# wvangansbeke/LaneDetection_End2End

Measured on AMD Instinct MI355X. Metric: images/sec fwd+bwd, 256x512 2-lane bs32, higher is better.
Workload: dtype f32; 1 GPU; BEV ERFNet + fused WLS fit + Area loss, 2 lanes, 256x512, batch 32 per GPU, fp32, train mode (BN batch stats, Dropout2d on), fwd+bwd, optimizer excluded; global_batch=32, parallelism=dp1, grad_allreduce=none

## Files before the change

lanedetection_end2end_amd/_lib.py:

```python
import ctypes
import os
from ctypes import c_char_p, c_double, c_int, c_long, c_size_t, c_void_p

import torch

_HERE = os.path.dirname(os.path.abspath(__file__))
LIB_PATH = os.path.join(_HERE, "liblanefit_hip.so")
_lib = None


class LaneFitLibraryError(RuntimeError):
    pass


def _declare(lib):
    P, I, L, D = c_void_p, c_int, c_long, c_double
    sig = {
        "lf_abi_version": (c_int, []),
        "lf_last_error": (c_char_p, []),
        "lf_wls_workspace_bytes": (c_size_t, [I, I, I]),
        "lf_wls_fwd": (I, [P, P, L, I, I, I, I, I, I, D, D, I, I, P, P, P, P, P, P]),
        "lf_wls_bwd": (I, [P, P, L, I, I, I, I, I, I, D, I, P, P, P, P, P]),
        "lf_gels_workspace_bytes": (c_size_t, [I, I]),
        "lf_gels_fwd": (I, [P, P, I, L, I, P, P, P, P, P]),
# ... 86 lines not shown
        "lf_wls_bwd_theta": (I, [P, P, L, P, P, I, I, I, I, I, I, D, I, P, P, P, P, P, P, P]),
        "lf_wls_bwd_grid": (I, [P, P, L, I, I, I, I, I, I, D, I, P, P, P, P, P]),
    }
    dbg = {
        "lf_debug_set_split_any_size": (None, [I]),
        "lf_debug_set_bf16_lds": (None, [I]),
        "lf_debug_set_ops_precision": (None, [I]),
        "lf_debug_conv1d_fwd_phases": (I, [P, P, P, P, I, I, I, I, I, I, P, P, P]),
        "lf_debug_conv1d_wgrad_phases": (I, [P, P, I, I, I, I, I, I, P, P, P]),
        "lf_debug_conv1d_fwd_pro": (I, [P, P, P, P, P, P, I, I, I, I, I, I, P, P]),
        "lf_debug_set_wgrad_ro": (None, [I, I, I]),
        "lf_debug_conv1d_bwd_data_epi3": (I, [P, P, P, P, P, P, P, I, I, I, I, I, I, P, P]),
        "lf_debug_conv1d_epi": (I, [P, P, P, P, I, I, P, P, P, P, P, P, I, I, I, I, I, I, P, P]),
        "lf_debug_conv1d_wgrad_pro": (I, [P, P, P, P, P, P, I, I, I, I, I, I, P, P]),
        "lf_debug_bias_residual_launches": (L, []),
    }
    for table in (sig, dbg):
        for name, (res, args) in table.items():
            fn = getattr(lib, name)
            fn.restype = res
            fn.argtypes = args
    return sig


def exported_symbols():
    return list(_declare(load()).keys()) + list(_extra_symbols)


_extra_symbols = []

# ... 56 lines not shown
```

lanedetection_end2end_amd/csrc/lf_conv.h:

```cpp
#pragma once
#include "lf_common.h"

#define LF_MAX_TAPS 9

struct LfTapGeom {
    int N, Hl, Wl;
    int Hs, Ws, s_pix, s_choff;
    int ssh, ssw;
    int Hd, Wd, d_pix, d_choff;
    int dsh, dsw, dah, daw;
    int Cs, Cd;
    int ntaps;
    int tdh[LF_MAX_TAPS], tdw[LF_MAX_TAPS];
};

enum { LF_PRO_NONE = 0, LF_PRO_BNRELU = 1 };
enum {
    LF_EPI_RELU = 1,
    LF_EPI_MASK = 2,
    LF_EPI_ADD = 4,
    LF_EPI_STATS_SQ = 8,
    LF_EPI_MASKBN = 16,
    LF_EPI_STATS_XHAT = 32,
    LF_EPI_BIAS = 64
// ... 17 lines not shown
    const float* msh;
    const float* asc;
    const float* ash;
    const float* dm;
    float* stats;
    int stats_ld;
    unsigned long long* dbg;
};

void lf_tapgemm_set_split_any_size(int v);
void lf_tapgemm_set_bf16_lds(int v);
int lf_tapgemm_stat_rows(const LfTapGeom& g);
int lf_tapgemm_stat_rows_for(const LfTapGeom& g, const LfTapArgs& a);
int lf_tapgemm_launch(const LfTapGeom& g, const LfTapArgs& a, int pro, int epi, hipStream_t st);
int lf_tapgemm_launch_unordered(const LfTapGeom& g, const LfTapArgs& a, int pro, int epi, hipStream_t st);

struct LfWgradArgs {
    const float* x;
    const float* g;
    const float* pro_sc;
    const float* pro_sh;
    int s16;
    int split;
    float* partial;
    float* bias_partial;
    unsigned long long* dbg = nullptr;
};
int lf_tapwgrad_splits(const LfTapGeom& g);
int lf_tapwgrad_splits_bound(const LfTapGeom& g, int s16);
int lf_tapwgrad_splits_for(const LfTapGeom& g, const LfWgradArgs& a, int pro);
// ... 53 lines not shown
```

lanedetection_end2end_amd/csrc/lf_conv.hip:

```cpp
#include <stdlib.h>
#include <string.h>

#include <atomic>
#include <map>
#include <mutex>
#include <tuple>
#include <utility>

#include <hip/hip_ext.h>

#include "lf_conv.h"
#include "lf_ldsdma.h"
#include "lf_types.h"

typedef float f32x4 __attribute__((ext_vector_type(4)));

namespace {

constexpr int MT = 4;
constexpr int WG_WAVES = 4;
constexpr int PIX_PER_WG = WG_WAVES * MT * 16;

__device__ __forceinline__ f32x4 ldg4(const float* p) { return *reinterpret_cast<const f32x4*>(p); }
typedef unsigned u32x4v __attribute__((vector_size(16)));
// ... 54 lines not shown
    r.x = dpp_mov<0x150>(v.x); r.y = dpp_mov<0x150>(v.y); r.z = dpp_mov<0x150>(v.z); r.w = dpp_mov<0x150>(v.w);
    return r;
}
__device__ __forceinline__ float sum16(float v) {
    v += dpp_mov<0xB1>(v);
    v += dpp_mov<0x4E>(v);
    v += dpp_mov<0x124>(v);
    v += dpp_mov<0x128>(v);
    return v;
}

#define LF_EPI_GROUPS 1
#define LF_EPI_ONE_TILE false
#define LF_EPI_TID threadIdx.x
#define LF_EPI_ROW1 false
#define LF_EPI_PIVOT true
#define LF_TAPGEMM_EPILOGUE \
      \
    const bool stats = (epi & (LF_EPI_STATS_SQ | LF_EPI_STATS_XHAT)) != 0; \
    constexpr bool NOBIAS = EPIC >= 0 && !(EPIC & LF_EPI_BIAS) && (EPIC & (LF_EPI_MASK | LF_EPI_ADD | LF_EPI_MASKBN | LF_EPI_STATS_XHAT)) != 0; \
    constexpr int NC = (NT % 2 == 0 && !LF_EPI_ONE_TILE) ? 2 : 1; \
     \
    constexpr bool HOISTM = HOISTV && !(EPIC >= 0 && (EPIC & LF_EPI_MASKBN) && (EPIC & LF_EPI_STATS_XHAT)); \
    __builtin_amdgcn_s_setprio(3);    \
    const __amdgpu_buffer_rsrc_t r_dst = make_rsrc(a.dst, 0xffffffffu), r_add = make_rsrc(a.add_src, 0xffffffffu), \
                                 r_msk = make_rsrc(a.mask_src, 0xffffffffu), r_aux = make_rsrc(a.aux, 0xffffffffu), \
                                 r_bias = make_rsrc(a.bias, 0xffffffffu), r_msc = make_rsrc(a.msc, 0xffffffffu), \
                                 r_msh = make_rsrc(a.msh, 0xffffffffu), r_dm = make_rsrc(a.dm, 0xffffffffu); \
     \
    f32x4 s1[NT], s2[NT], bs[NOBIAS ? 1 : NT], hv[HOISTV ? NT : 1][2], piv[LF_EPI_PIVOT ? NT : 1]; \
// ... 52 lines not shown
        for (int n = 0; n < NT; ++n) { \
            const f32x4 dmv = ldb4(r_dm, (unsigned)(pn[0] * g.Cd + cob + n * 16 + kq * 4) * 4u, 0u); \
            s1[n] *= dmv; s2[n] *= dmv; \
        } \
    } \
    if (stats) { \
         \
        const int EW = wave & 3, EG = wave >> 2; \
        __shared__ float sred[LF_EPI_GROUPS][WG_WAVES][NT][4][8]; \
_Pragma("unroll") \
        for (int n = 0; n < NT; ++n) { \
            f32x4 r1, r2; \
            r1.x = sum16(s1[n].x); r1.y = sum16(s1[n].y); r1.z = sum16(s1[n].z); r1.w = sum16(s1[n].w); \
            r2.x = sum16(s2[n].x); r2.y = sum16(s2[n].y); r2.z = sum16(s2[n].z); r2.w = sum16(s2[n].w); \
            if (epi & LF_EPI_STATS_SQ) {       \
                const unsigned lf_t0 = (bx * (unsigned)(WG_WAVES * LF_EPI_GROUPS) + (unsigned)wave) * 64u; \
                const float nw = lf_t0 < npix ? (float)min(npix - lf_t0, 64u) : 0.f; \
                const float rn = nw > 0.f ? 1.f / nw : 0.f; \
                r2 = r2 - r1 * r1 * rn; \
                r2.x = fmaxf(r2.x, 0.f); r2.y = fmaxf(r2.y, 0.f); r2.z = fmaxf(r2.z, 0.f); r2.w = fmaxf(r2.w, 0.f); \
                if (LF_EPI_PIVOT) r1 = r1 + piv[LF_EPI_PIVOT ? n : 0] * nw; \
            } \
            if (pl == 0) { \
                float* d = sred[EG][EW][n][kq]; \
                d[0] = r1.x; d[1] = r1.y; d[2] = r1.z; d[3] = r1.w; d[4] = r2.x; d[5] = r2.y; d[6] = r2.z; d[7] = r2.w; \
            } \
        } \
        __syncthreads(); \
        if ((LF_EPI_TID & 255) < NT * 4 * 8) { \
            const int tg = LF_EPI_TID >> 8, tt = LF_EPI_TID & 255; \
            const int j = tt & 7, q = (tt >> 3) & 3, n = tt >> 5; \
            float v = sred[tg][0][n][q][j] + sred[tg][1][n][q][j] + sred[tg][2][n][q][j] + sred[tg][3][n][q][j]; \
            if ((epi & LF_EPI_STATS_SQ) && j >= 4) {       \
                const unsigned lf_tb = (bx * (unsigned)LF_EPI_GROUPS + (unsigned)tg) * (unsigned)(WG_WAVES * 64); \
                float nwv[4], sw[4], nt = 0.f, st = 0.f; \
_Pragma("unroll") \
                for (int w = 0; w < 4; ++w) { \
                    const unsigned t0w = lf_tb + (unsigned)w * 64u; \
                    nwv[w] = t0w < npix ? (float)min(npix - t0w, 64u) : 0.f; \
                    sw[w] = sred[tg][w][n][q][j - 4]; \
                    nt += nwv[w]; st += sw[w]; \
                } \
                const float mg = nt > 0.f ? st / nt : 0.f; \
_Pragma("unroll") \
                for (int w = 0; w < 4; ++w) \
                    if (nwv[w] > 0.f) { const float dmw = sw[w] / nwv[w] - mg; v += nwv[w] * dmw * dmw; } \
            } \
            const int co = cob + n * 16 + q * 4 + (j & 3); \
            a.stats[((long)(j >> 2) * g.Cd + co) * a.stats_ld + ((long)bx * LF_EPI_GROUPS + tg)] = v;       \
        } \
    } \

extern __shared__ __attribute__((aligned(16))) unsigned char lf_tap_lds[];
constexpr size_t LF_TAP_LDS_PER_TAP = (size_t)WG_WAVES * 64 * (sizeof(uint4) + sizeof(unsigned));
// ... 1553 lines not shown
                for (int n = 0; n < NT; ++n)
#pragma unroll
                    for (int m = 0; m < MT; ++m)
                        seg[n][m] = __builtin_amdgcn_mfma_f32_16x16x4f32(w[n][s], x[m][s], seg[n][m], 0, 0, 0);
        }
    }
    if (!(g.Cs == 16 && g.ntaps == 3)) {
#pragma unroll
        for (int n = 0; n < NT; ++n)
#pragma unroll
            for (int m = 0; m < MT; ++m) acc[n][m] += seg[n][m];
    }
    LF_TAPGEMM_EPILOGUE
}

int g_split_any_size = 0;
std::atomic<long> g_bres_launches{0};
int g_bf16_lds = 4;

int pick_nt(int Cd) {
    const int tiles = Cd / 16;
    if (tiles % 4 == 0) return 4;
    if (tiles % 3 == 0) return 3;
    if (tiles % 2 == 0) return 2;
    return 1;
}

}

void lf_tapgemm_set_split_any_size(int v) { g_split_any_size = v; }
long lf_tapgemm_bias_residual_launches() { return g_bres_launches.load(); }
void lf_tapgemm_set_bf16_lds(int v) { g_bf16_lds = v; }

bool lf_tapgemm_split_ok(const LfTapGeom& g) {
    const long npix = (long)g.N * g.Hl * g.Wl;
    const long wgs = npix / (2 * PIX_PER_WG) * (g.Cd / 64);
    return g.Cs % 32 == 0 && g.Cd % 64 == 0 && g.s_pix % 4 == 0 && g.s_choff % 4 == 0 && npix % (2 * PIX_PER_WG) == 0 &&
           (wgs >= 192 || g_split_any_size);
}

int lf_tapgemm_stat_rows(const LfTapGeom& g) {
    const long npix = (long)g.N * g.Hl * g.Wl;
    return lf_cdiv(npix, PIX_PER_WG);
}
int lf_tapgemm_stat_rows_for(const LfTapGeom& g, const LfTapArgs& a) {
    (void)a;
    return lf_cdiv((long)g.N * g.Hl * g.Wl, PIX_PER_WG);
// ... 291 lines not shown
            if (pro == LF_PRO_BNRELU && epi == LF_EPI_RELU) LF_TG4(1, LF_EPI_RELU);
            else if (pro == LF_PRO_BNRELU) LF_TG4(1, -1);
            else switch (epis) {
                case 0: LF_TG4(0, 0); break;
                case LF_EPI_RELU: LF_TG4(0, LF_EPI_RELU); break;
                case LF_EPI_MASK: LF_TG4(0, LF_EPI_MASK); break;
                case LF_EPI_ADD: LF_TG4(0, LF_EPI_ADD); break;
                case LF_EPI_STATS_SQ: LF_TG4(0, LF_EPI_STATS_SQ); break;
                case LF_EPI_MASK | LF_EPI_STATS_XHAT: LF_TG4(0, LF_EPI_MASK | LF_EPI_STATS_XHAT); break;
                case LF_EPI_ADD | LF_EPI_MASK | LF_EPI_STATS_XHAT: LF_TG4(0, LF_EPI_ADD | LF_EPI_MASK | LF_EPI_STATS_XHAT); break;
                case LF_EPI_MASKBN | LF_EPI_STATS_XHAT: LF_TG4(0, LF_EPI_MASKBN | LF_EPI_STATS_XHAT); break;
                case BRES: LF_TG4(0, BRES); ++g_bres_launches; break;
                default: LF_TG4(0, -1); break;
            }
            break;
        case 3: LF_TG(3); break;
        case 2: LF_TG(2); break;
        default:
            {
#define LF_LEAN(PROV, EPIV) hipLaunchKernelGGL((tapgemm_lean_kernel<1, PROV, EPIV>), grid, dim3(256), 0, st, g, a, pro, epi)
                if (pro == LF_PRO_BNRELU && epi == LF_EPI_RELU) LF_LEAN(1, LF_EPI_RELU);
                else if (pro == LF_PRO_BNRELU) LF_LEAN(1, -1);
                else switch (epis) {
                    case 0: LF_LEAN(0, 0); break;
                    case LF_EPI_RELU: LF_LEAN(0, LF_EPI_RELU); break;
                    case LF_EPI_MASK: LF_LEAN(0, LF_EPI_MASK); break;
                    case LF_EPI_ADD: LF_LEAN(0, LF_EPI_ADD); break;
                    case LF_EPI_STATS_SQ: LF_LEAN(0, LF_EPI_STATS_SQ); break;
                    case LF_EPI_MASK | LF_EPI_STATS_XHAT: LF_LEAN(0, LF_EPI_MASK | LF_EPI_STATS_XHAT); break;
                    case LF_EPI_ADD | LF_EPI_MASK | LF_EPI_STATS_XHAT: LF_LEAN(0, LF_EPI_ADD | LF_EPI_MASK | LF_EPI_STATS_XHAT); break;
                    case LF_EPI_MASKBN | LF_EPI_STATS_XHAT: LF_LEAN(0, LF_EPI_MASKBN | LF_EPI_STATS_XHAT); break;
                    case BRES: LF_LEAN(0, BRES); ++g_bres_launches; break;
                    default: LF_LEAN(0, -1); break;
                }
#undef LF_LEAN
            }
            break;
    }
#undef LF_TG
#undef LF_TG4
    LF_CHECK_LAUNCH("tapgemm");
    return 0;
}

namespace {

template <bool S16>
__device__ __forceinline__ f32x4 wg_ld4(__amdgpu_buffer_rsrc_t r, unsigned off) { return epi_ld<S16>(r, off); }
template <bool S16>
__device__ __forceinline__ float wg_ld1(__amdgpu_buffer_rsrc_t r, unsigned off, unsigned soff = 0u) {
    if constexpr (S16) return __uint_as_float((unsigned)__builtin_amdgcn_raw_buffer_load_b16(r, (int)(off * 2u), (int)(soff * 2u), 0) << 16);
    else return __builtin_bit_cast(float, __builtin_amdgcn_raw_buffer_load_b32(r, (int)(off * 4u), (int)(soff * 4u), 0));
}
__device__ __forceinline__ uint2 wg_ldraw(__amdgpu_buffer_rsrc_t r, unsigned off) {
    return __builtin_bit_cast(uint2, __builtin_amdgcn_raw_buffer_load_b64(r, (int)(off * 2u), 0, 0));
}
// ... 1092 lines not shown
```

lanedetection_end2end_amd/csrc/lf_debug.h:

```cpp
#pragma once
#ifdef __cplusplus
extern "C" {
#endif
void lf_debug_set_split_any_size(int v);
void lf_debug_set_bf16_lds(int v);
void lf_debug_set_ops_precision(int mode);
int lf_debug_conv1d_fwd_phases(const float* x, const float* w, const float* bias, float* y, int N, int H, int W, int C,
                               int axis, int dilation, float* scratch, unsigned long long* dbg, void* stream);
int lf_debug_conv1d_fwd_pro(const float* x, const float* w, const float* bias, const float* sc, const float* sh, float* y, int N, int H,
                            int W, int C, int axis, int dilation, float* scratch, void* stream);
void lf_debug_set_wgrad_ro(int mode, int cap64, int cap128);
int lf_debug_conv1d_wgrad_pro(const float* x, const float* gy, const float* sc, const float* sh, float* gw, float* gb, int N, int H, int W,
                              int C, int axis, int dilation, float* scratch, void* stream);
int lf_debug_conv1d_bwd_data_epi3(const float* gy, const float* w, const float* mask_src, const float* add_src, const float* aux,
                                  float* gx, float* stats, int N, int H, int W, int C, int axis, int dilation, float* scratch, void* stream);
int lf_debug_conv1d_epi(const float* src, const float* w, const float* bias, float* dst, int transposed, int epi, const float* mask_src,
                        const float* add_src, const float* aux, const float* msc, const float* msh, float* stats, int N, int H, int W, int C,
                        int axis, int dilation, float* scratch, void* stream);
long lf_debug_bias_residual_launches(void);
int lf_debug_conv1d_wgrad_phases(const float* x, const float* gy, int N, int H, int W, int C, int axis, int dilation,
                                 float* scratch, unsigned long long* dbg, void* stream);
#ifdef __cplusplus
}
#endif
// ... 1 lines not shown
```

lanedetection_end2end_amd/csrc/lf_erfnet.hip:

```cpp
#include <stdlib.h>

#include <vector>

#include "lf_conv.h"
#include "lf_eltwise.h"
#include "lf_plan.h"
#include "lf_types.h"

namespace {

constexpr float BN_EPS = 1e-3f, BN_MOM = 0.1f;
enum { K_DOWN = 0, K_NB = 1, K_UP = 2 };

struct GemmOp {
    LfTapGeom geom;
    int pack;
};
struct BNRef {
    int p_g, p_b, idx, C;
    long sc, sh, asc, ash, c1, c2;
};
struct ConvRef {
    int p_w, p_b;
    GemmOp fwd;
// ... 280 lines not shown
    };
    auto add_up = [&](int cin, int cout) {
        Layer L;
        memset(&L, 0, sizeof(L));
        L.kind = K_UP; L.Cin = cin; L.Cout = cout; L.Hin = h; L.Win = w; L.Hout = 2 * h; L.Wout = 2 * w; L.drop_idx = -1;
        L.x = cur; L.reg_lo = ws.cur;
        L.cv[0].p_w = param++; L.cv[0].p_b = param++;
        L.bn[0].p_g = param++; L.bn[0].p_b = param++; L.bn[0].idx = bn++; L.bn[0].C = cout;
        const long sz = (long)N * 2 * h * 2 * w * cout;
        L.b[0] = ws.take(sz); L.b[1] = ws.take(sz);
        bn_alloc(ws, L.bn[0]);
        build_up_conv(P, L.cv[0], N, h, w, cin, cout);
        long rows4 = 0;
        for (int ph = 0; ph < 4; ++ph) { rows4 += lf_tapgemm_stat_rows(L.cv[0].fph[ph].geom); account_wgrad(P, L.cv[0].fph[ph].geom); }
        P->stat_floats = lf_maxl(P->stat_floats, rows4 * 2 * cout);
        P->layers.push_back(L);
        cur = L.b[1]; h *= 2; w *= 2;
    };
    add_down(in_channels, 16);
    add_down(16, 64);
    for (int i = 0; i < 5; ++i) add_nb(64, 0.03f, 1);
    add_down(64, 128);
    const int dils[8] = {2, 4, 8, 16, 2, 4, 8, 16};
    for (int i = 0; i < 8; ++i) add_nb(128, 0.3f, dils[i]);
    param += 2;
    add_up(128, 64);
    add_nb(64, 0.f, 1); add_nb(64, 0.f, 1);
    add_up(64, 16);
    add_nb(16, 0.f, 1); add_nb(16, 0.f, 1);
    for (int i = 0; i < n_heads; ++i) { P->p_head_w[i] = param++; P->p_head_b[i] = param++; }
// ... 122 lines not shown

int run_gemm(const Ctx& c, const GemmOp& op, const float* src, float* dst, const float* bias, int pro, int epi,
             LfTapArgs extra, bool beside_wgrad = false) {
    extra.src = src; extra.dst = dst; extra.bias = bias; extra.wp = c.packed(op.pack);
    extra.s16 = c.s16;
    if (c.P->precision == 2)
        extra.wp16 = reinterpret_cast<const unsigned short*>(c.at(c.P->off_packed16)) + c.P->packs[op.pack].dst16_off;
    if (c.P->precision == 3) {
        extra.split = 9;
        extra.wp48 = reinterpret_cast<const unsigned short*>(c.at(c.P->off_packed48)) + 3 * c.P->packs[op.pack].dst16_off;
    }
    c.last_rows = lf_tapgemm_stat_rows_for(op.geom, extra);
    ProfScope ps(c, 0, op.geom, epi | (pro << 8), c.st);
    if (beside_wgrad && c.wgrad_launched && !c.P->prof_on) return lf_tapgemm_launch_unordered(op.geom, extra, pro, epi, c.st);
    return lf_tapgemm_launch(op.geom, extra, pro, epi, c.st);
}

int bn_finalize(const Ctx& c, const BNRef& b, const LfStatPart* parts, int nparts, double count) {
    return lf_bn_finalize_fwd(parts, nparts, b.C, count, c.params[b.p_g], c.params[b.p_b], c.running[2 * b.idx],
                              c.running[2 * b.idx + 1], BN_MOM, BN_EPS, c.training, c.at(b.sc), c.at(b.sh), c.at(b.asc),
                              c.at(b.ash), c.st);
}

int encoder_layers(const lf_erfnet_plan* P) {
    int n = 0;
    for (const Layer& L : P->layers) { if (L.kind == K_UP) break; ++n; }
    return n;
}

int forward_layers(const Ctx& c, const float* img, int nlayers, int first = 0) {
// ... 40 lines not shown
            a = lf_no_args();
            a.pro_sc = c.at(L.bn[0].sc); a.pro_sh = c.at(L.bn[0].sh);
            LF_TRY(run_gemm(c, L.cv[2].fwd, c.at(L.b[1]), c.at(L.b[2]), c.params[L.cv[2].p_b], LF_PRO_BNRELU, LF_EPI_RELU, a));
            a = lf_no_args();
            a.stats = stat0; a.stats_ld = lf_stat_ld(lf_tapgemm_stat_rows(L.cv[3].fwd.geom));
            LF_TRY(run_gemm(c, L.cv[3].fwd, c.at(L.b[2]), c.at(L.b[3]), c.params[L.cv[3].p_b], LF_PRO_NONE,
                            c.training ? LF_EPI_STATS_SQ : 0, a));
            p0.nrows = p0.seg_rows = c.last_rows; p0.ld = a.stats_ld;
            LF_TRY(bn_finalize(c, L.bn[1], &p0, 1, (double)npo));
            const float* dm = (c.training && L.drop_idx >= 0 && c.dropmask) ? c.dropmask + P->drop_off[L.drop_idx] : nullptr;
            LF_TRY(lf_bn_act(c.at(L.b[3]), c.at(L.bn[1].sc), c.at(L.bn[1].sh), dm, c.at(L.x), c.at(L.b[4]), npo, L.Cout,
                             (long)L.Hout * L.Wout, c.s16, c.st));
        } else {
            LfStatPart parts[1];
            int rows = 0, rows4 = 0;
            for (int ph = 0; ph < 4; ++ph) rows4 += lf_tapgemm_stat_rows(L.cv[0].fph[ph].geom);
            for (int ph = 0; ph < 4; ++ph) {
                LfTapArgs a = lf_no_args();
                a.stats = stat0 + rows; a.stats_ld = lf_stat_ld(rows4);
                LF_TRY(run_gemm(c, L.cv[0].fph[ph], c.at(L.x), c.at(L.b[0]), c.params[L.cv[0].p_b], LF_PRO_NONE,
                                c.training ? LF_EPI_STATS_SQ : 0, a));
                rows += c.last_rows;
            }
            parts[0] = lf_stat_part_tiles(stat0, rows, lf_stat_ld(rows4), L.Cout, 0, rows / 4, npo / 4);
            LF_TRY(bn_finalize(c, L.bn[0], parts, 1, (double)npo));
            LF_TRY(lf_bn_act(c.at(L.b[0]), c.at(L.bn[0].sc), c.at(L.bn[0].sh), nullptr, nullptr, c.at(L.b[1]), npo, L.Cout,
                             (long)L.Hout * L.Wout, c.s16, c.st));
        }
    }
    return 0;
}

struct BiasChain { float* base = nullptr; int rows = 0; int phase = 0; };

int run_wgrad(const Ctx& c, const GemmOp& op, const ConvRef& cv, const float* x, const float* g, const float* pro_sc,
              const float* pro_sh, int bias_accumulate, bool batch_off = false, BiasChain* chain = nullptr) {
    const lf_erfnet_plan* P = c.P;
    c.wgrad_launched = false;
    if (!c.grads[cv.p_w]) return 0;
// ... 192 lines not shown
            add_prep(a, epi, L.cv[0].dg[0].geom);
            LF_TRY(run_gemm(c, L.cv[0].dg[0], X, F, nullptr, LF_PRO_NONE, epi, a));
            out = F;
            if (can_prep) { prepped = true; prep_rows = c.last_rows; prep_ld = a.stats_ld; }
        } else if (L.x < 0) {
            const int Cc = 16 - L.Cin, rows = lf_stem_wgrad_rows(N, L.Hin, L.Win);
            if (c.grads[L.cv[0].p_w]) {
                const RowSums rs = row_sum_regions(c, (long)rows * Cc * L.Cin * 9, (long)rows * Cc);
                LF_TRY(lf_stem_wgrad(img, X, N, L.Cin, L.Hin, L.Win, rs.wrows, rs.brows, c.s16, c.st));
                LF_TRY(row_sums_finish(c, rs, rows, Cc * L.Cin * 9, c.grads[L.cv[0].p_w], Cc, c.grads[L.cv[0].p_b]));
            }
            out = F;
        } else {
            LF_TRY(run_wgrad(c, L.cv[0].fwd, L.cv[0], c.at(L.x), X, nullptr, nullptr, 0));
            LF_TRY(lf_pool_bwd(c.at(L.x), X, N, L.Hin, L.Win, L.Cin, L.Cout, L.Cout - L.Cin, F, c.s16, c.st));
            for (int ph = 0; ph < 4; ++ph) {
                LfTapArgs a = lf_no_args();
                a.add_src = F;
                LF_TRY(run_gemm(c, L.cv[0].dg[ph], X, F, nullptr, LF_PRO_NONE, LF_EPI_ADD, a));
            }
            out = F;
        }
        in = out;
    }
    if (gin) *gin = in;
    return 0;
}

int upload_and_pack(const Ctx& c, const float* const* params_dev) {
    const lf_erfnet_plan* P = c.P;
    LfPackEntry* ent = reinterpret_cast<LfPackEntry*>(c.at(P->off_entries));
// ... 440 lines not shown
```

lanedetection_end2end_amd/csrc/lf_ops.hip:

```cpp
#include "lf_conv.h"
#include "lf_debug.h"

namespace {

__global__ __launch_bounds__(256) void pack_one_kernel(const float* __restrict__ w, float* __restrict__ dst, int Kc, int Nc,
                                                      int ntaps, long sk, long sn, int flip) {
    const long total = (long)ntaps * Kc * Nc;
    for (long i = (long)blockIdx.x * 256 + threadIdx.x; i < total; i += (long)gridDim.x * 256) {
        const int k4 = (int)(i & 3);
        long r = i >> 2;
        const int n = (int)(r % Nc);
        r /= Nc;
        const int kb = (int)(r % (Kc >> 2));
        const int t = (int)(r / (Kc >> 2));
        dst[i] = w[(kb * 4 + k4) * sk + n * sn + (flip ? ntaps - 1 - t : t)];
    }
}

__global__ __launch_bounds__(256) void pack_one_bf16_kernel(const float* __restrict__ w, __bf16* __restrict__ dst, int Kc, int Nc,
                                                           int ntaps, long sk, long sn, int flip) {
    const int kb_per_tap = ((Kc + 31) >> 5) * 4;
    const long total = (long)ntaps * kb_per_tap * Nc * 8;
    for (long i = (long)blockIdx.x * 256 + threadIdx.x; i < total; i += (long)gridDim.x * 256) {
        const int k8 = (int)(i & 7);
// ... 36 lines not shown
            hipLaunchKernelGGL(pack_one_split_kernel, dim3(64), dim3(256), 0, st, w, reinterpret_cast<__bf16*>(scratch + 3L * C * C),
                               C, C, 3, sk, sn, flip);
            a.split = g_ops_bf16;
            a.wp48 = scratch + 3L * C * C;
        }
    } else if (g_ops_bf16 == 2) {
        hipLaunchKernelGGL(pack_one_bf16_kernel, dim3(64), dim3(256), 0, st, w, reinterpret_cast<__bf16*>(scratch), C, C, 3, sk, sn, flip);
        a.wp16 = scratch;
        a.s16 = 1;
    } else {
        hipLaunchKernelGGL(pack_one_kernel, dim3(64), dim3(256), 0, st, w, scratch, C, C, 3, sk, sn, flip);
    }
    a.wp = scratch;
}

LfTapGeom conv1d_geom(int N, int H, int W, int C, int axis, int d) {
    LfTapGeom g;
    memset(&g, 0, sizeof(g));
    g.N = N; g.Hl = H; g.Wl = W; g.Hs = H; g.Ws = W; g.s_pix = C; g.ssh = 1; g.ssw = 1;
    g.Hd = H; g.Wd = W; g.d_pix = C; g.dsh = 1; g.dsw = 1; g.Cs = C; g.Cd = C; g.ntaps = 3;
    for (int t = 0; t < 3; ++t) { g.tdh[t] = axis == 0 ? (t - 1) * d : 0; g.tdw[t] = axis == 1 ? (t - 1) * d : 0; }
    return g;
}

}

extern "C" {

void lf_debug_set_split_any_size(int v) { lf_tapgemm_set_split_any_size(v); }
void lf_debug_set_bf16_lds(int v) { lf_tapgemm_set_bf16_lds(v); }
void lf_debug_set_ops_precision(int mode) { g_ops_bf16 = (mode == 2 || mode == 9) ? mode : 0; }

void lf_debug_set_wgrad_ro(int mode, int cap64, int cap128) { lf_tapwgrad_ro_set(mode, cap64, cap128); }
long lf_debug_bias_residual_launches(void) { return lf_tapgemm_bias_residual_launches(); }

int lf_debug_conv1d_fwd_phases(const float* x, const float* w, const float* bias, float* y, int N, int H, int W, int C,
                               int axis, int dilation, float* scratch, unsigned long long* dbg, void* stream) {
    hipStream_t st = (hipStream_t)stream;
    const LfTapGeom g = conv1d_geom(N, H, W, C, axis, dilation);
    LfTapArgs a;
    memset(&a, 0, sizeof(a));
    pack_conv1d(a, w, scratch, C, 3L, 3L * C, 0, st);
    a.src = x; a.bias = bias; a.dst = y; a.dbg = dbg;
    return lf_tapgemm_launch(g, a, LF_PRO_NONE, 0, st);
}

// ... 116 lines not shown
```

Baseline: 1992 images/sec.

## Fuse four transposed-conv phase GEMMs into one kernel sharing input loads

Adds a phase4 kernel that computes all four sub-pixel phases of the stride-2 transposed convolution (upsampler) in one launch. It walks the 9 taps in an order that reuses each input pixel load across phases, and keeps four accumulator sets in registers. It is used for the forward pass with BN stats and for the backward data-grad with the add epilogue when fp32 and the geometry qualifies. It also specialises the 3-tap conv1d stats kernel on width alignment. The cost is higher register pressure from four accumulator sets, and separate stats tiling for the fused path.

New measurement: 2004 images/sec, median of 6. Within noise of the previous version (+0.6%).

```diff
diff --git a/lanedetection_end2end_amd/_lib.py b/lanedetection_end2end_amd/_lib.py
--- a/lanedetection_end2end_amd/_lib.py
+++ b/lanedetection_end2end_amd/_lib.py
@@ -124,6 +124,8 @@
         "lf_debug_conv1d_epi": (I, [P, P, P, P, I, I, P, P, P, P, P, P, I, I, I, I, I, I, P, P]),
         "lf_debug_conv1d_wgrad_pro": (I, [P, P, P, P, P, P, I, I, I, I, I, I, P, P]),
         "lf_debug_bias_residual_launches": (L, []),
+        "lf_debug_set_phase_fused": (None, [I]),
+        "lf_debug_phase4": (I, [P, P, P, P, P, P, I, I, I, I, I, I, I, P, P]),
     }
     for table in (sig, dbg):
         for name, (res, args) in table.items():
diff --git a/lanedetection_end2end_amd/csrc/lf_conv.h b/lanedetection_end2end_amd/csrc/lf_conv.h
--- a/lanedetection_end2end_amd/csrc/lf_conv.h
+++ b/lanedetection_end2end_amd/csrc/lf_conv.h
@@ -55,6 +55,13 @@
 int lf_tapgemm_stat_rows_for(const LfTapGeom& g, const LfTapArgs& a);
 int lf_tapgemm_launch(const LfTapGeom& g, const LfTapArgs& a, int pro, int epi, hipStream_t st);
 int lf_tapgemm_launch_unordered(const LfTapGeom& g, const LfTapArgs& a, int pro, int epi, hipStream_t st);
+
+struct LfPhase4 { unsigned woff[4]; int rows_per_phase; };
+bool lf_tapgemm_phase4_ok(const LfTapGeom* g, const LfTapArgs& a, const float* const* wp, int pro, int epi);
+int lf_tapgemm_phase4_tile_pix(const LfTapGeom& g0);
+int lf_tapgemm_phase4_stat_rows(const LfTapGeom& g0);
+int lf_tapgemm_phase4_launch(const LfTapGeom* g, const LfTapArgs& a, const float* const* wp, int epi, hipStream_t st);
+void lf_tapgemm_set_phase_fused(int v);
 
 struct LfWgradArgs {
     const float* x;
diff --git a/lanedetection_end2end_amd/csrc/lf_conv.hip b/lanedetection_end2end_amd/csrc/lf_conv.hip
--- a/lanedetection_end2end_amd/csrc/lf_conv.hip
+++ b/lanedetection_end2end_amd/csrc/lf_conv.hip
@@ -92,6 +92,7 @@
 #define LF_EPI_ONE_TILE false
 #define LF_EPI_TID threadIdx.x
 #define LF_EPI_ROW1 false
+#define LF_EPI_WPIX 64u
 #define LF_EPI_PIVOT true
 #define LF_TAPGEMM_EPILOGUE \
       \
@@ -174,8 +175,8 @@
             r1.x = sum16(s1[n].x); r1.y = sum16(s1[n].y); r1.z = sum16(s1[n].z); r1.w = sum16(s1[n].w); \
             r2.x = sum16(s2[n].x); r2.y = sum16(s2[n].y); r2.z = sum16(s2[n].z); r2.w = sum16(s2[n].w); \
             if (epi & LF_EPI_STATS_SQ) {       \
-                const unsigned lf_t0 = (bx * (unsigned)(WG_WAVES * LF_EPI_GROUPS) + (unsigned)wave) * 64u; \
-                const float nw = lf_t0 < npix ? (float)min(npix - lf_t0, 64u) : 0.f; \
+                const unsigned lf_t0 = (bx * (unsigned)(WG_WAVES * LF_EPI_GROUPS) + (unsigned)wave) * LF_EPI_WPIX; \
+                const float nw = lf_t0 < npix ? (float)min(npix - lf_t0, LF_EPI_WPIX) : 0.f; \
                 const float rn = nw > 0.f ? 1.f / nw : 0.f; \
                 r2 = r2 - r1 * r1 * rn; \
                 r2.x = fmaxf(r2.x, 0.f); r2.y = fmaxf(r2.y, 0.f); r2.z = fmaxf(r2.z, 0.f); r2.w = fmaxf(r2.w, 0.f); \
@@ -192,12 +193,12 @@
             const int j = tt & 7, q = (tt >> 3) & 3, n = tt >> 5; \
             float v = sred[tg][0][n][q][j] + sred[tg][1][n][q][j] + sred[tg][2][n][q][j] + sred[tg][3][n][q][j]; \
             if ((epi & LF_EPI_STATS_SQ) && j >= 4) {       \
-                const unsigned lf_tb = (bx * (unsigned)LF_EPI_GROUPS + (unsigned)tg) * (unsigned)(WG_WAVES * 64); \
+                const unsigned lf_tb = (bx * (unsigned)LF_EPI_GROUPS + (unsigned)tg) * ((unsigned)WG_WAVES * LF_EPI_WPIX); \
                 float nwv[4], sw[4], nt = 0.f, st = 0.f; \
 _Pragma("unroll") \
                 for (int w = 0; w < 4; ++w) { \
-                    const unsigned t0w = lf_tb + (unsigned)w * 64u; \
-                    nwv[w] = t0w < npix ? (float)min(npix - t0w, 64u) : 0.f; \
+                    const unsigned t0w = lf_tb + (unsigned)w * LF_EPI_WPIX; \
+                    nwv[w] = t0w < npix ? (float)min(npix - t0w, LF_EPI_WPIX) : 0.f; \
                     sw[w] = sred[tg][w][n][q][j - 4]; \
                     nt += nwv[w]; st += sw[w]; \
                 } \
@@ -1781,8 +1782,128 @@
     LF_TAPGEMM_EPILOGUE
 }
 
+template <int NTC, int EPIC>
+__global__ __launch_bounds__(256, 2) void tapgemm_phase4_kernel(const LfTapGeom g0, const LfTapArgs a0, const LfPhase4 pw) {
+    constexpr int NT = NTC, MT = 4 / NTC;
+    constexpr bool S16 = false, HOISTV = true;
+    const int epi = EPIC;
+    const int cob = 0;
+    const unsigned npix = (unsigned)(g0.N * g0.Hl * g0.Wl);
+    unsigned bx = blockIdx.x;
+    if ((gridDim.x & 7u) == 0) bx = (bx & 7u) * (gridDim.x >> 3) + (bx >> 3);
+    const int lane = threadIdx.x & 63, wave = threadIdx.x >> 6;
+    const int pl = lane & 15, kq = lane >> 4;
+    const unsigned tile0 = (bx * WG_WAVES + (unsigned)wave) * (MT * 16);
+    int pn[MT], pi[MT], pj[MT];
+    bool pv[MT];
+    unsigned xb[MT];
+#pragma unroll
+    for (int m = 0; m < MT; ++m) {
+        const unsigned p = tile0 + m * 16 + pl;
+        pv[m] = p < npix;
+        const unsigned q = pv[m] ? p : 0u;
+        const unsigned r = q / (unsigned)g0.Wl;
+        pj[m] = (int)(q - r * (unsigned)g0.Wl);
+        pn[m] = (int)(r / (unsigned)g0.Hl);
+        pi[m] = (int)(r - (unsigned)pn[m] * (unsigned)g0.Hl);
+        xb[m] = (unsigned)(((pn[m] * g0.Hs + pi[m]) * g0.Ws + pj[m]) * g0.s_pix + g0.s_choff + kq * 4) * 4u;
+    }
+    f32x4 accP[4][NT][MT], acclP[4][NT][MT];
+#pragma unroll
+    for (int ph = 0; ph < 4; ++ph)
+#pragma unroll
+        for (int n = 0; n < NT; ++n)
+#pragma unroll
+            for (int m = 0; m < MT; ++m) { accP[ph][n][m] = zero4(); acclP[ph][n][m] = zero4(); }
+    const int ncg = g0.Cs >> 4;
+    const __amdgpu_buffer_rsrc_t rx = make_rsrc(a0.src, (unsigned)min((long)g0.N * g0.Hs * g0.Ws * g0.s_pix * 4, (long)LF_OOB));
+    const __amdgpu_buffer_rsrc_t rw = make_rsrc(a0.wp, 0xffffffffu);
+    const unsigned wlane = (unsigned)(kq * g0.Cd + pl) * 16u;
+    const unsigned wstep = (unsigned)g0.Cd * 64u;
+#define LF_P4_XOFF(DST, DY, DX)                                                                              \
+    _Pragma("unroll") for (int m = 0; m < MT; ++m) {                                                          \
+        const bool in = pv[m] && pi[m] + (DY) < g0.Hs && pj[m] + (DX) < g0.Ws;                                \
+        DST[m] = in ? xb[m] + (unsigned)(((DY) * g0.Ws + (DX)) * g0.s_pix) * 4u : LF_OOB;                     \
+    }
+    f32x4 wc[NT], xc[MT];
+    {
+        unsigned xo[MT];
+        LF_P4_XOFF(xo, 1, 1)
+#pragma unroll
+        for (int n = 0; n < NT; ++n) wc[n] = ldb4(rw, wlane + n * 256, pw.woff[3]);
+#pragma unroll
+        for (int m = 0; m < MT; ++m) xc[m] = ldb4(rx, xo[m], 0u);
+    }
+#define LF_P4_TAP(PH, TAPI, DY, DX, PHN, TAPIN, DYN, DXN)                                                     \
+    {                                                                                                         \
+        unsigned xo[MT], xon[MT];                                                                             \
+        LF_P4_XOFF(xo, DY, DX)                                                                                \
+        LF_P4_XOFF(xon, DYN, DXN)                                                                             \
+        const unsigned wb = pw.woff[PH] + (unsigned)((TAPI) * ncg) * wstep;                                   \
+        const unsigned wbn = pw.woff[PHN] + (unsigned)((TAPIN) * ncg) * wstep;                                \
+        for (int cg = 0; cg < ncg; ++cg) {                                                                    \
+            const bool last = cg + 1 == ncg;                                                                  \
+            const unsigned wso = last ? wbn : wb + (unsigned)(cg + 1) * wstep;                                \
+            const unsigned c16 = last ? 0u : (unsigned)(cg + 1) * 64u;                                        \
+            f32x4 wn[NT], xn[MT];                                                                             \
+            _Pragma("unroll") for (int n = 0; n < NT; ++n) wn[n] = ldb4(rw, wlane + n * 256, wso);            \
+            _Pragma("unroll") for (int m = 0; m < MT; ++m) xn[m] = ldb4(rx, last ? xon[m] : xo[m], c16);      \
+            if (!(cg & 1)) {       \
+                _Pragma("unroll") for (int n = 0; n < NT; ++n)                                                \
+                    _Pragma("unroll") for (int m = 0; m < MT; ++m) {                                          \
+                        acclP[PH][n][m] += accP[PH][n][m];                                                    \
+                        accP[PH][n][m] = zero4();                                                             \
+                    }                                                                                         \
+            }                                                                                                 \
+            _Pragma("unroll") for (int s4 = 0; s4 < 4; ++s4)                                                  \
+                _Pragma("unroll") for (int n = 0; n < NT; ++n)                                                \
+                    _Pragma("unroll") for (int m = 0; m < MT; ++m)                                            \
+                        accP[PH][n][m] = __builtin_amdgcn_mfma_f32_16x16x4f32(wc[n][s4], xc[m][s4], accP[PH][n][m], 0, 0, 0); \
+            _Pragma("unroll") for (int n = 0; n < NT; ++n) wc[n] = wn[n];                                     \
+            _Pragma("unroll") for (int m = 0; m < MT; ++m) xc[m] = xn[m];                                     \
+        }                                                                                                     \
+    }
+    LF_P4_TAP(3, 0, 1, 1, 3, 1, 1, 0)
+    LF_P4_TAP(3, 1, 1, 0, 2, 0, 1, 0)
+    LF_P4_TAP(2, 0, 1, 0, 3, 2, 0, 1)
+    LF_P4_TAP(3, 2, 0, 1, 1, 0, 0, 1)
+    LF_P4_TAP(1, 0, 0, 1, 3, 3, 0, 0)
+    LF_P4_TAP(3, 3, 0, 0, 2, 1, 0, 0)
+    LF_P4_TAP(2, 1, 0, 0, 1, 1, 0, 0)
+    LF_P4_TAP(1, 1, 0, 0, 0, 0, 0, 0)
+    LF_P4_TAP(0, 0, 0, 0, 0, 0, 0, 0)
+#undef LF_P4_TAP
+#undef LF_P4_XOFF
+#pragma unroll
+    for (int ph = 0; ph < 4; ++ph)
+#pragma unroll
+        for (int n = 0; n < NT; ++n)
+#pragma unroll
+            for (int m = 0; m < MT; ++m) accP[ph][n][m] += acclP[ph][n][m];
+#undef LF_EPI_WPIX
+#define LF_EPI_WPIX ((unsigned)(MT * 16))
+#define LF_P4_EPI(PH)                                                                                         \
+    {                                                                                                         \
+        LfTapGeom g = g0;                                                                                     \
+        g.dah = (PH) >> 1; g.daw = (PH) & 1;                                                                  \
+        LfTapArgs a = a0;                                                                                     \
+        a.stats = a0.stats + (long)(PH) * pw.rows_per_phase;                                                  \
+        f32x4 (&acc)[NT][MT] = accP[PH];                                                                      \
+        LF_TAPGEMM_EPILOGUE                                                                                   \
+    }
+    LF_P4_EPI(0)
+    LF_P4_EPI(1)
+    LF_P4_EPI(2)
+    LF_P4_EPI(3)
+#undef LF_P4_EPI
+#undef LF_EPI_WPIX
+#define LF_EPI_WPIX 64u
+    __builtin_amdgcn_s_setprio(0);
+}
+
 int g_split_any_size = 0;
 std::atomic<long> g_bres_launches{0};
+int g_phase_fused = 1;
 int g_bf16_lds = 4;
 
 int pick_nt(int Cd) {
@@ -1798,6 +1919,7 @@
 void lf_tapgemm_set_split_any_size(int v) { g_split_any_size = v; }
 long lf_tapgemm_bias_residual_launches() { return g_bres_launches.load(); }
 void lf_tapgemm_set_bf16_lds(int v) { g_bf16_lds = v; }
+void lf_tapgemm_set_phase_fused(int v) { g_phase_fused = v; }
 
 bool lf_tapgemm_split_ok(const LfTapGeom& g) {
     const long npix = (long)g.N * g.Hl * g.Wl;
@@ -2119,7 +2241,12 @@
                 default: LF_TG4(0, -1); break;
             }
             break;
-        case 3: LF_TG(3); break;
+        case 3:
+            if (pro == LF_PRO_NONE && epis == LF_EPI_STATS_SQ) {
+                if ((g.Wl & 63) == 0) launch_tapgemm(tapgemm_kernel<3, 0, LF_EPI_STATS_SQ, true>, grid, tap_lds, st, g, a, pro, epi);
+                else launch_tapgemm(tapgemm_kernel<3, 0, LF_EPI_STATS_SQ, false>, grid, tap_lds, st, g, a, pro, epi);
+            } else LF_TG(3);
+            break;
         case 2: LF_TG(2); break;
         default:
             {
@@ -2145,6 +2272,50 @@
 #undef LF_TG
 #undef LF_TG4
     LF_CHECK_LAUNCH("tapgemm");
+    return 0;
+}
+
+int lf_tapgemm_phase4_tile_pix(const LfTapGeom& g0) { return g0.Cd == 64 ? 64 : 256; }
+int lf_tapgemm_phase4_stat_rows(const LfTapGeom& g0) { return lf_cdiv((long)g0.N * g0.Hl * g0.Wl, lf_tapgemm_phase4_tile_pix(g0)); }
+bool lf_tapgemm_phase4_ok(const LfTapGeom* g, const LfTapArgs& a, const float* const* wp, int pro, int epi) {
+    if (!g_phase_fused || a.s16 || a.wp16 || a.split || a.dbg || pro != LF_PRO_NONE) return false;
+    if (!(epi == 0 || epi == LF_EPI_STATS_SQ || (epi == LF_EPI_ADD && !a.bias))) return false;
+    const LfTapGeom& g0 = g[0];
+    if (!((g0.Cd == 64 && g0.Cs % 32 == 0) || (g0.Cd == 16 && g0.Cs % 16 == 0)) || g0.Wl % 16 != 0) return false;
+    if (g0.s_pix % 4 || g0.s_choff % 4 || g0.d_pix % 4 || g0.d_choff % 4) return false;
+    if ((long)g0.N * g0.Hs * g0.Ws * g0.s_pix * 4 >= (long)LF_OOB || (long)g0.N * g0.Hd * g0.Wd * g0.d_pix * 4 >= (long)LF_OOB) return false;
+    if ((long)g0.N * g0.Hl * g0.Wl >= (1L << 30)) return false;
+    static const int ntap[4] = {1, 2, 2, 4};
+    static const int dy[4][4] = {{0}, {0, 0}, {1, 0}, {1, 1, 0, 0}}, dx[4][4] = {{0}, {1, 0}, {0, 0}, {1, 0, 1, 0}};
+    for (int ph = 0; ph < 4; ++ph) {
+        const LfTapGeom& p = g[ph];
+        if (p.N != g0.N || p.Hl != g0.Hl || p.Wl != g0.Wl || p.Hs != p.Hl || p.Ws != p.Wl || p.ssh != 1 || p.ssw != 1 || p.dsh != 2 ||
+            p.dsw != 2 || p.Hd != 2 * p.Hl || p.Wd != 2 * p.Wl || p.dah != (ph >> 1) || p.daw != (ph & 1) || p.s_pix != g0.s_pix ||
+            p.s_choff != g0.s_choff || p.d_pix != g0.d_pix || p.d_choff != g0.d_choff || p.Cs != g0.Cs || p.Cd != g0.Cd || p.ntaps != ntap[ph])
+            return false;
+        for (int t = 0; t < p.ntaps; ++t)
+            if (p.tdh[t] != dy[ph][t] || p.tdw[t] != dx[ph][t]) return false;
+        if (wp[ph] < wp[0] || (wp[ph] - wp[0]) * 4L >= (1L << 30)) return false;
+    }
+    return true;
+}
+int lf_tapgemm_phase4_launch(const LfTapGeom* g, const LfTapArgs& a0, const float* const* wp, int epi, hipStream_t st) {
+    LfTapArgs a = a0;
+    LF_REQUIRE(lf_tapgemm_phase4_ok(g, a, wp, LF_PRO_NONE, epi), "tapgemm_phase4: launch not qualified (geometry, epilogue %d or precision)", epi);
+    LfPhase4 pw;
+    for (int ph = 0; ph < 4; ++ph) pw.woff[ph] = (unsigned)((wp[ph] - wp[0]) * 4L);
+    pw.rows_per_phase = lf_tapgemm_phase4_stat_rows(g[0]);
+    a.wp = wp[0];
+    const dim3 grid(pw.rows_per_phase);
+#define LF_P4(NTV)                                                                                                              \
+    do {                                                                                                                        \
+        if (epi == 0) hipLaunchKernelGGL((tapgemm_phase4_kernel<NTV, 0>), grid, dim3(256), 0, st, g[0], a, pw);                  \
+        else if (epi == LF_EPI_ADD) hipLaunchKernelGGL((tapgemm_phase4_kernel<NTV, LF_EPI_ADD>), grid, dim3(256), 0, st, g[0], a, pw); \
+        else hipLaunchKernelGGL((tapgemm_phase4_kernel<NTV, LF_EPI_STATS_SQ>), grid, dim3(256), 0, st, g[0], a, pw);             \
+    } while (0)
+    if (g[0].Cd == 64) LF_P4(4); else LF_P4(1);
+#undef LF_P4
+    LF_CHECK_LAUNCH("tapgemm_phase4");
     return 0;
 }
 
diff --git a/lanedetection_end2end_amd/csrc/lf_debug.h b/lanedetection_end2end_amd/csrc/lf_debug.h
--- a/lanedetection_end2end_amd/csrc/lf_debug.h
+++ b/lanedetection_end2end_amd/csrc/lf_debug.h
@@ -4,6 +4,9 @@
 #endif
 void lf_debug_set_split_any_size(int v);
 void lf_debug_set_bf16_lds(int v);
+void lf_debug_set_phase_fused(int v);
+int lf_debug_phase4(const float* src, const float* w, const float* bias, float* dst, const float* add_src, float* stats, int epi, int N,
+                    int H, int W, int Ck, int Cn, int s_pix, float* scratch, void* stream);
 void lf_debug_set_ops_precision(int mode);
 int lf_debug_conv1d_fwd_phases(const float* x, const float* w, const float* bias, float* y, int N, int H, int W, int C,
                                int axis, int dilation, float* scratch, unsigned long long* dbg, void* stream);
diff --git a/lanedetection_end2end_amd/csrc/lf_erfnet.hip b/lanedetection_end2end_amd/csrc/lf_erfnet.hip
--- a/lanedetection_end2end_amd/csrc/lf_erfnet.hip
+++ b/lanedetection_end2end_amd/csrc/lf_erfnet.hip
@@ -318,6 +318,7 @@
         long rows4 = 0;
         for (int ph = 0; ph < 4; ++ph) { rows4 += lf_tapgemm_stat_rows(L.cv[0].fph[ph].geom); account_wgrad(P, L.cv[0].fph[ph].geom); }
         P->stat_floats = lf_maxl(P->stat_floats, rows4 * 2 * cout);
+        P->stat_floats = lf_maxl(P->stat_floats, 4L * lf_tapgemm_phase4_stat_rows(L.cv[0].fph[0].geom) * 2 * cout);
         P->layers.push_back(L);
         cur = L.b[1]; h *= 2; w *= 2;
     };
@@ -470,6 +471,22 @@
     ProfScope ps(c, 0, op.geom, epi | (pro << 8), c.st);
     if (beside_wgrad && c.wgrad_launched && !c.P->prof_on) return lf_tapgemm_launch_unordered(op.geom, extra, pro, epi, c.st);
     return lf_tapgemm_launch(op.geom, extra, pro, epi, c.st);
+}
+
+int run_phase4(const Ctx& c, const GemmOp* ops, const float* src, float* dst, const float* bias, int epi, LfTapArgs extra, bool* fused) {
+    *fused = false;
+    if (c.P->precision != 0) return 0;
+    extra.src = src; extra.dst = dst; extra.bias = bias; extra.s16 = c.s16;
+    LfTapGeom g[4];
+    const float* wp[4];
+    for (int ph = 0; ph < 4; ++ph) { g[ph] = ops[ph].geom; wp[ph] = c.packed(ops[ph].pack); }
+    if (!lf_tapgemm_phase4_ok(g, extra, wp, LF_PRO_NONE, epi)) return 0;
+    *fused = true;
+    LfTapGeom gp = g[0];
+    gp.ntaps = 9;
+    c.last_rows = 4 * lf_tapgemm_phase4_stat_rows(g[0]);
+    ProfScope ps(c, 0, gp, epi, c.st);
+    return lf_tapgemm_phase4_launch(g, extra, wp, epi, c.st);
 }
 
 int bn_finalize(const Ctx& c, const BNRef& b, const LfStatPart* parts, int nparts, double count) {
@@ -540,15 +557,23 @@
         } else {
             LfStatPart parts[1];
             int rows = 0, rows4 = 0;
+            bool fused = false;
+            {
+                LfTapArgs a = lf_no_args();
+                a.stats = stat0; a.stats_ld = lf_stat_ld(4 * lf_tapgemm_phase4_stat_rows(L.cv[0].fph[0].geom));
+                LF_TRY(run_phase4(c, L.cv[0].fph, c.at(L.x), c.at(L.b[0]), c.params[L.cv[0].p_b], c.training ? LF_EPI_STATS_SQ : 0, a, &fused));
+                if (fused) parts[0] = lf_stat_part_tiles(stat0, c.last_rows, a.stats_ld, L.Cout, 0, c.last_rows / 4, npo / 4,
+                                                         lf_tapgemm_phase4_tile_pix(L.cv[0].fph[0].geom));
+            }
             for (int ph = 0; ph < 4; ++ph) rows4 += lf_tapgemm_stat_rows(L.cv[0].fph[ph].geom);
-            for (int ph = 0; ph < 4; ++ph) {
+            for (int ph = 0; ph < 4 && !fused; ++ph) {
                 LfTapArgs a = lf_no_args();
                 a.stats = stat0 + rows; a.stats_ld = lf_stat_ld(rows4);
                 LF_TRY(run_gemm(c, L.cv[0].fph[ph], c.at(L.x), c.at(L.b[0]), c.params[L.cv[0].p_b], LF_PRO_NONE,
                                 c.training ? LF_EPI_STATS_SQ : 0, a));
                 rows += c.last_rows;
             }
-            parts[0] = lf_stat_part_tiles(stat0, rows, lf_stat_ld(rows4), L.Cout, 0, rows / 4, npo / 4);
+            if (!fused) parts[0] = lf_stat_part_tiles(stat0, rows, lf_stat_ld(rows4), L.Cout, 0, rows / 4, npo / 4);
             LF_TRY(bn_finalize(c, L.bn[0], parts, 1, (double)npo));
             LF_TRY(lf_bn_act(c.at(L.b[0]), c.at(L.bn[0].sc), c.at(L.bn[0].sh), nullptr, nullptr, c.at(L.b[1]), npo, L.Cout,
                              (long)L.Hout * L.Wout, c.s16, c.st));
@@ -771,7 +796,13 @@
         } else {
             LF_TRY(run_wgrad(c, L.cv[0].fwd, L.cv[0], c.at(L.x), X, nullptr, nullptr, 0));
             LF_TRY(lf_pool_bwd(c.at(L.x), X, N, L.Hin, L.Win, L.Cin, L.Cout, L.Cout - L.Cin, F, c.s16, c.st));
-            for (int ph = 0; ph < 4; ++ph) {
+            bool fused = false;
+            {
+                LfTapArgs a = lf_no_args();
+                a.add_src = F;
+                LF_TRY(run_phase4(c, L.cv[0].dg, X, F, nullptr, LF_EPI_ADD, a, &fused));
+            }
+            for (int ph = 0; ph < 4 && !fused; ++ph) {
                 LfTapArgs a = lf_no_args();
                 a.add_src = F;
                 LF_TRY(run_gemm(c, L.cv[0].dg[ph], X, F, nullptr, LF_PRO_NONE, LF_EPI_ADD, a));
diff --git a/lanedetection_end2end_amd/csrc/lf_ops.hip b/lanedetection_end2end_amd/csrc/lf_ops.hip
--- a/lanedetection_end2end_amd/csrc/lf_ops.hip
+++ b/lanedetection_end2end_amd/csrc/lf_ops.hip
@@ -74,6 +74,21 @@
     a.wp = scratch;
 }
 
+__global__ __launch_bounds__(256) void pack_taps_kernel(const float* __restrict__ w, float* __restrict__ dst, int Kc, int Nc, int ntaps,
+                                                       long sk, long sn, int4 tapidx) {
+    const long total = (long)ntaps * Kc * Nc;
+    for (long i = (long)blockIdx.x * 256 + threadIdx.x; i < total; i += (long)gridDim.x * 256) {
+        const int k4 = (int)(i & 3);
+        long r = i >> 2;
+        const int n = (int)(r % Nc);
+        r /= Nc;
+        const int kb = (int)(r % (Kc >> 2));
+        const int t = (int)(r / (Kc >> 2));
+        const int ti = t == 0 ? tapidx.x : t == 1 ? tapidx.y : t == 2 ? tapidx.z : tapidx.w;
+        dst[i] = w[(kb * 4 + k4) * sk + n * sn + ti];
+    }
+}
+
 LfTapGeom conv1d_geom(int N, int H, int W, int C, int axis, int d) {
     LfTapGeom g;
     memset(&g, 0, sizeof(g));
@@ -90,6 +105,48 @@
 void lf_debug_set_split_any_size(int v) { lf_tapgemm_set_split_any_size(v); }
 void lf_debug_set_bf16_lds(int v) { lf_tapgemm_set_bf16_lds(v); }
 void lf_debug_set_ops_precision(int mode) { g_ops_bf16 = (mode == 2 || mode == 9) ? mode : 0; }
+
+void lf_debug_set_phase_fused(int v) { lf_tapgemm_set_phase_fused(v); }
+
+int lf_debug_phase4(const float* src, const float* w, const float* bias, float* dst, const float* add_src, float* stats, int epi, int N,
+                    int H, int W, int Ck, int Cn, int s_pix, float* scratch, void* stream) {
+    if (!(src && w && dst && scratch)) { lf_fail("lf_debug_phase4: null pointer"); return -1; }
+    hipStream_t st = (hipStream_t)stream;
+    LfTapGeom g[4];
+    const float* wp[4];
+    float* next = scratch;
+    for (int a = 0; a < 2; ++a)
+        for (int b = 0; b < 2; ++b) {
+            LfTapGeom& p = g[a * 2 + b];
+            memset(&p, 0, sizeof(p));
+            p.N = N; p.Hl = H; p.Wl = W; p.Hs = H; p.Ws = W; p.s_pix = s_pix; p.ssh = 1; p.ssw = 1;
+            p.Hd = 2 * H; p.Wd = 2 * W; p.d_pix = Cn; p.dsh = 2; p.dsw = 2; p.dah = a; p.daw = b; p.Cs = Ck; p.Cd = Cn;
+            const int na = a ? 2 : 1, nb = b ? 2 : 1;
+            const int kh[2] = {a ? 0 : 1, 2}, oh[2] = {a ? 1 : 0, 0}, kw[2] = {b ? 0 : 1, 2}, ow[2] = {b ? 1 : 0, 0};
+            int ti[4] = {0, 0, 0, 0};
+            for (int i = 0; i < na; ++i)
+                for (int j = 0; j < nb; ++j) { p.tdh[p.ntaps] = oh[i]; p.tdw[p.ntaps] = ow[j]; ti[p.ntaps] = kh[i] * 3 + kw[j]; ++p.ntaps; }
+            hipLaunchKernelGGL(pack_taps_kernel, dim3(64), dim3(256), 0, st, w, next, Ck, Cn, p.ntaps, (long)Cn * 9, 9L,
+                               make_int4(ti[0], ti[1], ti[2], ti[3]));
+            wp[a * 2 + b] = next;
+            next += (long)p.ntaps * Ck * Cn;
+        }
+    LfTapArgs args;
+    memset(&args, 0, sizeof(args));
+    args.src = src; args.dst = dst; args.bias = bias; args.add_src = add_src; args.stats = stats;
+    if (lf_tapgemm_phase4_ok(g, args, wp, LF_PRO_NONE, epi)) {
+        const int rows = lf_tapgemm_phase4_stat_rows(g[0]);
+        args.stats_ld = 4 * rows;
+        return lf_tapgemm_phase4_launch(g, args, wp, epi, st) ? -1 : rows;
+    }
+    const int rows = lf_tapgemm_stat_rows(g[0]);
+    for (int ph = 0; ph < 4; ++ph) {
+        LfTapArgs a1 = args;
+        a1.wp = wp[ph]; a1.stats = stats ? stats + (long)ph * rows : nullptr; a1.stats_ld = 4 * rows;
+        if (lf_tapgemm_launch(g[ph], a1, LF_PRO_NONE, epi, st)) return -1;
+    }
+    return rows;
+}
 
 void lf_debug_set_wgrad_ro(int mode, int cap64, int cap128) { lf_tapwgrad_ro_set(mode, cap64, cap128); }
 long lf_debug_bias_residual_launches(void) { return lf_tapgemm_bias_residual_launches(); }
```
